# SeanNaren/deepspeech.pytorch

Measured on AMD Instinct MI355X. Metric: audio-seconds/sec (train step), higher is better.
Workload: dtype bf16

## Files before the change

deepspeech/pytorch_amd/csrc/ds2_gemm8.hip:

```cpp
#include "ds2_common.h"

namespace {

typedef __attribute__((address_space(3))) void* lds_ptr_t;
typedef const __attribute__((address_space(1))) void* glb_ptr_t;

constexpr int G8_MAX_GROUPS = 6;

struct G8Problem {
  const bf16_t* A;
  const bf16_t* A2;
  const bf16_t* B;
  void* C;
  const float* bias;
  int M, N, m_split;
  long lda, lda2, ldb, ldc;
  int tiles_n, tile_end;
  int out_is_f32;
  int K, tn;
  const int* rows;
};
struct G8Args {
  G8Problem p[G8_MAX_GROUPS];
  int n_problems;
};

#define G8_WAIT_VM(n) asm volatile("s_waitcnt vmcnt(" #n ")" ::: "memory")
#define G8_WAIT_LGKM0() asm volatile("s_waitcnt lgkmcnt(0)" ::: "memory")
#define G8_BARRIER()                        \
  do {                                      \
    __builtin_amdgcn_sched_barrier(0);      \
    __builtin_amdgcn_s_barrier();           \
    __builtin_amdgcn_sched_barrier(0);      \
  } while (0)

template <bool TN, bool SPREAD>
__device__ __forceinline__ void g8_tile(const G8Problem& P, int t_id, unsigned char* lds) {
  const int tid = threadIdx.x, lane = tid & 63;
  const int wave = __builtin_amdgcn_readfirstlane(tid >> 6);
  const int wm = wave >> 2, wn = wave & 3;
#ifndef DS2_G8_SWZ
#define DS2_G8_SWZ 1
#endif
  int tm_ = t_id / P.tiles_n, tn_ = t_id % P.tiles_n;
  if (DS2_G8_SWZ > 1 && P.tiles_n > 32 / DS2_G8_SWZ) {
    const int tiles_m = ((TN ? P.M : P.M) + 255) / 256;
    const int per = DS2_G8_SWZ * P.tiles_n, st = t_id / per, wi = t_id - st * per;
    const int rows = min(DS2_G8_SWZ, tiles_m - st * DS2_G8_SWZ);
    tm_ = st * DS2_G8_SWZ + wi % rows;
    tn_ = wi / rows;
  }
  const int m0 = tm_ * 256, n0 = tn_ * 256;
  const int K_ = P.K;
  const int nkt = (K_ + 63) / 64;
  const int krem = K_ - (nkt - 1) * 64;
  const bool tail = TN && krem < 64;

  ds2_f32x16 acc[4][2];
#pragma unroll
  for (int i = 0; i < 4; ++i)
#pragma unroll
    for (int j = 0; j < 2; ++j)
#pragma unroll
      for (int r = 0; r < 16; ++r) acc[i][j][r] = 0.f;

  uint32_t a_off[4], b_off[4];
  const bf16_t* a_base = P.A;
  const bf16_t* b_base = P.B;
  if constexpr (!TN) {
    const int rloc = wave * 8 + (lane >> 3);
    const int chunk = (lane & 7) ^ ((rloc >> 1) & 7);
#pragma unroll
    for (int rb = 0; rb < 4; ++rb) {
      int ar = min(m0 + rb * 64 + rloc, P.M - 1);
      if (P.rows) ar = P.rows[ar];
      a_off[rb] = (uint32_t)(((long)ar * P.lda + chunk * 8) * 2);
      b_off[rb] = (uint32_t)(((long)min(n0 + rb * 64 + rloc, P.N - 1) * P.ldb + chunk * 8) * 2);
    }
  } else {
#pragma unroll
    for (int rb = 0; rb < 4; ++rb) {
      const int kr = rb * 16 + wave * 2 + (lane >> 5);
      const int chunk = (lane & 31) ^ ((kr & 3) << 2);
      int mcol = m0 + chunk * 8, ncol = min(n0 + chunk * 8, P.N - 8);
      const int mlim = (P.A2 && m0 >= P.m_split) ? P.M - P.m_split : (P.A2 ? P.m_split : P.M);
      if (P.A2 && m0 >= P.m_split) mcol -= P.m_split;
      mcol = min(mcol, mlim - 8);
      a_off[rb] = (uint32_t)(((long)kr * ((P.A2 && m0 >= P.m_split) ? P.lda2 : P.lda) + mcol) * 2);
      b_off[rb] = (uint32_t)(((long)kr * P.ldb + ncol) * 2);
    }
    if (P.A2 && m0 >= P.m_split) a_base = P.A2;
  }
  const long lda_eff = (TN && P.A2 && m0 >= P.m_split) ? P.lda2 : P.lda;
  const int t_kr0 = wave * 2 + (lane >> 5);
  const uint32_t t_acol = TN ? a_off[0] - (uint32_t)((long)t_kr0 * ((P.A2 && m0 >= P.m_split) ? P.lda2 : P.lda) * 2) : 0;
  const uint32_t t_bcol = TN ? b_off[0] - (uint32_t)((long)t_kr0 * P.ldb * 2) : 0;
  const long a_kstep = TN ? 128 * lda_eff : 128, b_kstep = TN ? 128 * P.ldb : 128;
  const bool listed = TN && P.rows != nullptr;
  typedef const __attribute__((address_space(4))) int* const_int_ptr_t;
  const const_int_ptr_t crows = (const_int_ptr_t)(uintptr_t)P.rows;
  uint32_t rk[4] = {0, 0, 0, 0};
  int sr0[4] = {0, 0, 0, 0}, sr1[4] = {0, 0, 0, 0};
  auto fetch_rows = [&](int kt) {
    if (listed && kt < nkt) {
#pragma unroll
      for (int rb = 0; rb < 4; ++rb) {
        const int k = kt * 64 + rb * 16 + wave * 2;
        sr0[rb] = crows[min(k, K_ - 1)];
        sr1[rb] = crows[min(k + 1, K_ - 1)];
      }
    }
  };
  auto select_rows = [&]() {
    if (listed) {
#pragma unroll
      for (int rb = 0; rb < 4; ++rb) rk[rb] = (uint32_t)((lane >> 5) ? sr1[rb] : sr0[rb]);
    }
  };
  const uint32_t lda2b = (uint32_t)(lda_eff * 2), ldb2b = (uint32_t)(P.ldb * 2);
  auto stage_a = [&](int b, int kt, int r0 = 0, int r1 = 4) {
    const unsigned char* src = (const unsigned char*)a_base + (long)kt * a_kstep;
    unsigned char* d = lds + b * 32768 + wave * 1024;
    if (listed) {
#pragma unroll
      for (int rb = 0; rb < 4; ++rb)
        if (rb >= r0 && rb < r1)
          __builtin_amdgcn_global_load_lds((glb_ptr_t)((const unsigned char*)a_base + (size_t)(rk[rb] * lda2b + t_acol)), (lds_ptr_t)(d + rb * 8192), 16, 0, 0);
    } else if (tail && kt == nkt - 1) {
#pragma unroll
      for (int rb = 0; rb < 4; ++rb)
        if (rb >= r0 && rb < r1) {
          const uint32_t off = (uint32_t)((long)min(t_kr0 + rb * 16, krem - 1) * lda_eff * 2) + t_acol;
          __builtin_amdgcn_global_load_lds((glb_ptr_t)(src + (size_t)off), (lds_ptr_t)(d + rb * 8192), 16, 0, 0);
        }
    } else {
#pragma unroll
      for (int rb = 0; rb < 4; ++rb)
        if (rb >= r0 && rb < r1) __builtin_amdgcn_global_load_lds((glb_ptr_t)(src + (size_t)a_off[rb]), (lds_ptr_t)(d + rb * 8192), 16, 0, 0);
    }
  };
  auto stage_b = [&](int b, int kt, int r0 = 0, int r1 = 4) {
    const unsigned char* src = (const unsigned char*)b_base + (long)kt * b_kstep;
    unsigned char* d = lds + 65536 + b * 32768 + wave * 1024;
    if (listed) {
#pragma unroll
      for (int rb = 0; rb < 4; ++rb)
        if (rb >= r0 && rb < r1)
          __builtin_amdgcn_global_load_lds((glb_ptr_t)((const unsigned char*)b_base + (size_t)(rk[rb] * ldb2b + t_bcol)), (lds_ptr_t)(d + rb * 8192), 16, 0, 0);
    } else if (tail && kt == nkt - 1) {
#pragma unroll
      for (int rb = 0; rb < 4; ++rb)
        if (rb >= r0 && rb < r1) {
          const uint32_t off = (uint32_t)((long)min(t_kr0 + rb * 16, krem - 1) * P.ldb * 2) + t_bcol;
          __builtin_amdgcn_global_load_lds((glb_ptr_t)(src + (size_t)off), (lds_ptr_t)(d + rb * 8192), 16, 0, 0);
        }
    } else {
#pragma unroll
      for (int rb = 0; rb < 4; ++rb)
        if (rb >= r0 && rb < r1) __builtin_amdgcn_global_load_lds((glb_ptr_t)(src + (size_t)b_off[rb]), (lds_ptr_t)(d + rb * 8192), 16, 0, 0);
    }
  };
  auto zero_tail = [&](int b) {
    if (wm == 0) {
      const int nbytes = (64 - krem) * 512;
      for (int o = tid * 16; o < nbytes; o += 256 * 16) {
        *reinterpret_cast<uint4*>(lds + b * 32768 + krem * 512 + o) = make_uint4(0, 0, 0, 0);
        *reinterpret_cast<uint4*>(lds + 65536 + b * 32768 + krem * 512 + o) = make_uint4(0, 0, 0, 0);
      }
      G8_WAIT_LGKM0();
    }
    G8_BARRIER();
  };

  const int li = lane & 31, lq = lane >> 5;
  const uint32_t lds0 = (uint32_t)(uintptr_t)(__attribute__((address_space(3))) unsigned char*)lds;
  struct Frag {
    uint4 v;
    uint2 lo, hi;
  };
  Frag fa[2][4], fbx[4], fby[4];
  uint32_t ra[4], rb_[4];
  if constexpr (!TN) {
    const int key = (li >> 1) & 7;
#pragma unroll
    for (int c = 0; c < 4; ++c) {
      ra[c] = lds0 + (wm * 128 + li) * 128 + (((2 * c + lq) ^ key) << 4);
      rb_[c] = lds0 + 65536 + (wn * 64 + li) * 128 + (((2 * c + lq) ^ key) << 4);
    }
  } else {
    const int l16 = lane & 15, gq = lane >> 4;
    const int krow = 8 * (gq >> 1) + (l16 >> 2);
    const int mloc = 16 * (gq & 1) + 4 * (l16 & 3);
#pragma unroll
    for (int j = 0; j < 4; ++j) ra[j] = lds0 + krow * 512 + mloc * 2 + ((((wm * 4 + j) ^ (l16 >> 2))) << 6);
#pragma unroll
    for (int j = 0; j < 2; ++j) rb_[j] = lds0 + 65536 + krow * 512 + mloc * 2 + ((((wn * 2 + j) ^ (l16 >> 2))) << 6);
    rb_[2] = rb_[3] = 0;
  }
#define G8_RD128(dst, addr, off) asm volatile("ds_read_b128 %0, %1 offset:%2" : "=v"(dst) : "v"(addr), "i"(off))
#define G8_RDTR(dst, addr, off) asm volatile("ds_read_b64_tr_b16 %0, %1 offset:%2" : "=v"(dst) : "v"(addr), "i"(off))
#define G8_READ_A(BUF, MH)                                                                      \
  _Pragma("unroll") for (int i = 0; i < 2; ++i) _Pragma("unroll") for (int c = 0; c < 4; ++c) { \
    if constexpr (!TN) {                                                                        \
      G8_RD128(fa[i][c].v, ra[c], (BUF) * 32768 + ((MH) * 64 + i * 32) * 128);                  \
    } else {                                                                                    \
      G8_RDTR(fa[i][c].lo, ra[(MH) * 2 + i], (BUF) * 32768 + c * 8192);                         \
      G8_RDTR(fa[i][c].hi, ra[(MH) * 2 + i], (BUF) * 32768 + c * 8192 + 2048);                  \
    }                                                                                           \
  }
#define G8_READ_B(BUF, NH, FB)                                           \
  _Pragma("unroll") for (int c = 0; c < 4; ++c) {                        \
    if constexpr (!TN) {                                                 \
      G8_RD128(FB[c].v, rb_[c], (BUF) * 32768 + (NH) * 32 * 128);        \
    } else {                                                             \
      G8_RDTR(FB[c].lo, rb_[NH], (BUF) * 32768 + c * 8192);              \
      G8_RDTR(FB[c].hi, rb_[NH], (BUF) * 32768 + c * 8192 + 2048);       \
    }                                                                    \
  }
  auto frag = [&](const Frag& f) {
    if constexpr (!TN)
      return f.v;
    else
      return make_uint4(f.lo.x, f.lo.y, f.hi.x, f.hi.y);
  };
  auto mma = [&](int mh, int nh, const Frag (&fb)[4]) {
    __builtin_amdgcn_s_setprio(1);
#pragma unroll
    for (int c = 0; c < 4; ++c)
#pragma unroll
      for (int i = 0; i < 2; ++i)
        Mma<bf16_t>::mma32(acc[mh * 2 + i][nh], frag(fb[c]), frag(fa[i][c]));
    __builtin_amdgcn_s_setprio(0);
  };

#define G8_KTILE(BUF, KT)                                      \
  {                                                            \
    const bool more = (KT) + 2 < nkt;                          \
    const bool more_a = SPREAD && (KT) >= 1 && (KT) + 1 < nkt; \
    if (tail && (KT) == nkt - 1) zero_tail(BUF);               \
                                                  \
    fetch_rows((KT) + 2);                                      \
    G8_READ_A(BUF, 0)                                          \
    G8_READ_B(BUF, 0, fbx)                                     \
    if (more_a) stage_a((BUF) ^ 1, (KT) + 1, 0, 2);            \
    G8_BARRIER();                                              \
    G8_WAIT_LGKM0();                                           \
    __builtin_amdgcn_sched_barrier(0);                         \
    mma(0, 0, fbx);                                            \
    G8_BARRIER();                                              \
                                                  \
    G8_READ_B(BUF, 1, fby)                                     \
    if (more_a) stage_a((BUF) ^ 1, (KT) + 1, 2, 4);            \
    G8_WAIT_LGKM0();                                           \
    G8_BARRIER();                                              \
    mma(0, 1, fby);                                            \
    G8_BARRIER();                                              \
                                                  \
    G8_READ_A(BUF, 1)                                          \
    select_rows();                                             \
    if (more) stage_b(BUF, (KT) + 2, 0, SPREAD ? 2 : 4);       \
    G8_WAIT_LGKM0();                                           \
    G8_BARRIER();                                              \
    mma(1, 1, fby);                                            \
    G8_BARRIER();                                              \
                                                  \
    if (SPREAD) {                                              \
      if (more) {                                              \
        stage_b(BUF, (KT) + 2, 2, 4);                          \
        G8_WAIT_VM(4);                                         \
      } else {                                                 \
        G8_WAIT_VM(0);                                         \
      }                                                        \
    } else if (more) {                                         \
      stage_a(BUF, (KT) + 2);                                  \
      G8_WAIT_VM(8);                                           \
    } else {                                                   \
      G8_WAIT_VM(0);                                           \
    }                                                          \
    G8_BARRIER();                                              \
    mma(1, 0, fbx);                                            \
    G8_BARRIER();                                              \
  }

  fetch_rows(0);
  select_rows();
  stage_a(0, 0);
  stage_b(0, 0);
  if (nkt > 1) {
    fetch_rows(1);
    select_rows();
    stage_a(1, 1);
    stage_b(1, 1);
    G8_WAIT_VM(8);
  } else {
    G8_WAIT_VM(0);
  }
  G8_BARRIER();
  if (wm == 1) G8_BARRIER();
  for (int kt = 0; kt < nkt; kt += 2) {
    G8_KTILE(0, kt)
    if (kt + 1 < nkt) G8_KTILE(1, kt + 1)
  }
  if (wm == 0) G8_BARRIER();

  int eli = li, elq = lq;
  asm volatile("" : "+v"(eli), "+v"(elq));
  const float* bias = P.bias;
  const int M_ = P.M, N_ = P.N;
  const long ldc = P.ldc;
  if (!P.out_is_f32 && (ldc % 8 == 0) && ((((uintptr_t)P.C) & 15) == 0)) {
    unsigned char* ep = lds + wave * 9216;
    bf16_t* Cb = (bf16_t*)P.C;
#pragma unroll
    for (int half = 0; half < 2; ++half) {
#pragma unroll
      for (int i2 = 0; i2 < 2; ++i2)
#pragma unroll
        for (int j = 0; j < 2; ++j)
#pragma unroll
          for (int q = 0; q < 4; ++q) {
            const int col = j * 32 + 8 * q + 4 * elq;
            const int gcol = n0 + wn * 64 + col;
            float bv[4] = {0.f, 0.f, 0.f, 0.f};
            if (bias) {
#pragma unroll
              for (int e = 0; e < 4; ++e) bv[e] = gcol + e < N_ ? bias[gcol + e] : 0.f;
            }
            uint2 pk;
            pk.x = cvt_pk_bf16(acc[half * 2 + i2][j][4 * q + 0] + bv[0], acc[half * 2 + i2][j][4 * q + 1] + bv[1]);
            pk.y = cvt_pk_bf16(acc[half * 2 + i2][j][4 * q + 2] + bv[2], acc[half * 2 + i2][j][4 * q + 3] + bv[3]);
            *reinterpret_cast<uint2*>(ep + (i2 * 32 + eli) * 144 + col * 2) = pk;
          }
#pragma unroll
      for (int r = 0; r < 8; ++r) {
        const int row_l = r * 8 + (lane >> 3), seg = lane & 7;
        const uint4 d = *reinterpret_cast<const uint4*>(ep + row_l * 144 + seg * 16);
        const int grow = m0 + wm * 128 + half * 64 + row_l, gcol = n0 + wn * 64 + seg * 8;
        if (grow < M_) {
          bf16_t* cp = Cb + (long)(P.rows ? P.rows[grow] : grow) * ldc + gcol;
          if (gcol + 7 < N_) {
            *reinterpret_cast<uint4*>(cp) = d;
          } else {
            const uint32_t w[4] = {d.x, d.y, d.z, d.w};
#pragma unroll
            for (int e = 0; e < 8; ++e)
              if (gcol + e < N_) cp[e].v = (uint16_t)(w[e >> 1] >> ((e & 1) * 16));
          }
        }
      }
    }
    return;
  }
  const bool n_vec_ok = (ldc % 4 == 0);
#pragma unroll
  for (int i = 0; i < 4; ++i) {
    const int row = m0 + wm * 128 + i * 32 + eli;
    if (row >= M_) continue;
#pragma unroll
    for (int j = 0; j < 2; ++j) {
#pragma unroll
      for (int q = 0; q < 4; ++q) {
        const int col = n0 + wn * 64 + j * 32 + 8 * q + 4 * elq;
        if (col >= N_) continue;
        float v[4];
#pragma unroll
        for (int e = 0; e < 4; ++e) v[e] = acc[i][j][4 * q + e] + ((bias && col + e < N_) ? bias[col + e] : 0.f);
        const long off = (long)((!TN && P.rows) ? P.rows[row] : row) * ldc + col;
        if (P.out_is_f32) {
          float* cp = (float*)P.C + off;
          if (col + 3 < N_ && n_vec_ok) {
            *reinterpret_cast<float4*>(cp) = make_float4(v[0], v[1], v[2], v[3]);
          } else {
#pragma unroll
            for (int e = 0; e < 4; ++e)
              if (col + e < N_) cp[e] = v[e];
          }
        } else {
          bf16_t* cp = (bf16_t*)P.C + off;
#pragma unroll
          for (int e = 0; e < 4; ++e)
            if (col + e < N_) stf(cp + e, v[e]);
        }
      }
    }
  }
}


template <int MODE, bool SPREAD>
__global__ void __launch_bounds__(512, 2) k_gemm8(G8Args g) {
  __shared__ __attribute__((aligned(1024))) unsigned char lds[131072];
  const int id = blockIdx.x;
  int pi = 0, first = 0;
#pragma unroll
  for (int i = 0; i < G8_MAX_GROUPS - 1; ++i)
    if (i + 1 < g.n_problems && id >= g.p[i].tile_end) {
      pi = i + 1;
      first = g.p[i].tile_end;
    }
  const G8Problem& P = g.p[pi];
  const int count = P.tile_end - first, local = id - first, xcd = id & 7;
  int base = 0;
#pragma unroll
  for (int y = 0; y < 8; ++y) {
    const int l0 = (y - first) & 7;
    const int n_y = l0 < count ? (count - l0 - 1) / 8 + 1 : 0;
    if (y < xcd) base += n_y;
  }
  const int t_id = base + (local - ((xcd - first) & 7)) / 8;
  if (MODE == 0)
    g8_tile<false, SPREAD>(P, t_id, lds);
  else if (MODE == 1)
    g8_tile<true, SPREAD>(P, t_id, lds);
  else if (P.tn)
    g8_tile<true, SPREAD>(P, t_id, lds);
  else
    g8_tile<false, SPREAD>(P, t_id, lds);
}

template <int MODE>
void g8_launch(int total, const G8Args& g, hipStream_t st) {
  hipLaunchKernelGGL((k_gemm8<MODE, false>), dim3(total), dim3(512), 0, st, g);
}

}


static int g8_nt(const void* A, const void* B, void* C, const float* bias, int M, int N, int K, long lda, long ldb, long ldc, int out_f32,
                 const int* rows, int n_phys, hipStream_t st) {
  DS2_REQUIRE(M > 0 && N > 0 && K > 0 && K % 64 == 0 && lda % 8 == 0 && ldb % 8 == 0 && n_phys >= M, DS2_ERR_ARG);
  DS2_REQUIRE((((uintptr_t)A) & 15) == 0 && (((uintptr_t)B) & 15) == 0, DS2_ERR_ALIGN);
  DS2_REQUIRE((long)n_phys * lda < (1L << 31) && (long)N * ldb < (1L << 31), DS2_ERR_ARG);
  G8Args g{};
  g.n_problems = 1;
  const int tm = ds2_cdiv(M, 256), tn = ds2_cdiv(N, 256);
  g.p[0] = G8Problem{(const bf16_t*)A, nullptr, (const bf16_t*)B, C, bias, M, N, 0, lda, 0, ldb, ldc, tn, tm * tn, out_f32, K, 0, rows};
  g8_launch<0>(tm * tn, g, st);
  DS2_CHECK_LAUNCH();
  return 0;
}

static int g8_tn_fill(G8Args& g, int& total, int n, const void* const* At, const void* const* At2, const int* m_split, const void* const* Bt,
                      void* const* C, const int* M, const int* N, const long* lda, const long* lda2, const long* ldb, const long* ldc, int K,
                      const int* rows, int n_phys) {
  DS2_REQUIRE(K > 0 && n_phys >= K, DS2_ERR_ARG);
  for (int i = 0; i < n; ++i) {
    DS2_REQUIRE(M[i] > 0 && N[i] > 0 && M[i] % 8 == 0 && N[i] % 8 == 0 && lda[i] % 8 == 0 && ldb[i] % 8 == 0, DS2_ERR_ARG);
    DS2_REQUIRE((((uintptr_t)At[i]) & 15) == 0 && (((uintptr_t)Bt[i]) & 15) == 0, DS2_ERR_ALIGN);
    DS2_REQUIRE((long)n_phys * lda[i] < (1L << 31) && (long)n_phys * ldb[i] < (1L << 31), DS2_ERR_ARG);
    const void* a2 = At2 ? At2[i] : nullptr;
    const int ms = a2 ? m_split[i] : 0;
    DS2_REQUIRE(a2 == nullptr || (ms > 0 && ms < M[i] && ms % 256 == 0 && (((uintptr_t)a2) & 15) == 0 && lda2 && lda2[i] % 8 == 0 &&
                                  (long)n_phys * lda2[i] < (1L << 31)), DS2_ERR_ARG);
    const int tm = ds2_cdiv(M[i], 256), tn = ds2_cdiv(N[i], 256);
    total += tm * tn;
    g.p[i] = G8Problem{(const bf16_t*)At[i], (const bf16_t*)a2, (const bf16_t*)Bt[i], C[i], nullptr, M[i], N[i], ms, lda[i], a2 ? lda2[i] : 0, ldb[i], ldc[i], tn, total, 1, K, 1, rows};
  }
  return 0;
}

extern "C" {

int ds2_gemm8_nt(const void* A, const void* B, void* C, const float* bias, int M, int N, int K, long lda, long ldb, long ldc, int out_f32,
                 ds2_stream_t st) {
  return g8_nt(A, B, C, bias, M, N, K, lda, ldb, ldc, out_f32, nullptr, M, (hipStream_t)st);
}
int ds2_gemm8_nt_rows(const void* A, const void* B, void* C, const float* bias, int n_phys, int N, int K, long lda, long ldb, long ldc,
                      int out_f32, const int* rows, int n_rows, ds2_stream_t st) {
  return g8_nt(A, B, C, bias, rows ? n_rows : n_phys, N, K, lda, ldb, ldc, out_f32, rows, n_phys, (hipStream_t)st);
}

int ds2_gemm8_tn_grouped_rows(int n_problems, const void* const* At, const void* const* At2, const int* m_split, const void* const* Bt,
                              void* const* C, const int* M, const int* N, const long* lda, const long* lda2, const long* ldb, const long* ldc,
                              int n_phys, const int* rows, int n_rows, ds2_stream_t st) {
  DS2_REQUIRE(n_problems >= 1 && n_problems <= G8_MAX_GROUPS, DS2_ERR_ARG);
  G8Args g{};
  g.n_problems = n_problems;
  int total = 0;
  const int rc = g8_tn_fill(g, total, n_problems, At, At2, m_split, Bt, C, M, N, lda, lda2, ldb, ldc, rows ? n_rows : n_phys, rows, n_phys);
  if (rc) return rc;
  g8_launch<1>(total, g, (hipStream_t)st);
  DS2_CHECK_LAUNCH();
  return 0;
}
int ds2_gemm8_tn_grouped(int n_problems, const void* const* At, const void* const* At2, const int* m_split, const void* const* Bt, void* const* C,
                         const int* M, const int* N, const long* lda, const long* lda2, const long* ldb, const long* ldc, int K, ds2_stream_t st) {
  return ds2_gemm8_tn_grouped_rows(n_problems, At, At2, m_split, Bt, C, M, N, lda, lda2, ldb, ldc, K, nullptr, K, st);
}

int ds2_gemm8_wgrad_dx_rows(int n_tn, const void* const* At, const void* const* At2, const int* m_split, const void* const* Bt, void* const* C,
                            const int* M, const int* N, const long* lda, const long* lda2, const long* ldb, const long* ldc, int K_tn,
                            const void* A_nt, const void* B_nt, void* C_nt, int M_nt, int N_nt, int K_nt, long lda_nt, long ldb_nt, long ldc_nt,
                            const int* rows, int n_rows, ds2_stream_t st) {
  DS2_REQUIRE(n_tn >= 1 && n_tn < G8_MAX_GROUPS && K_tn > 0, DS2_ERR_ARG);
  DS2_REQUIRE(rows == nullptr || (K_tn == M_nt && n_rows > 0 && n_rows <= K_tn), DS2_ERR_ARG);
  DS2_REQUIRE(M_nt > 0 && N_nt > 0 && K_nt > 0 && K_nt % 64 == 0 && lda_nt % 8 == 0 && ldb_nt % 8 == 0, DS2_ERR_ARG);
  DS2_REQUIRE((((uintptr_t)A_nt) & 15) == 0 && (((uintptr_t)B_nt) & 15) == 0, DS2_ERR_ALIGN);
  DS2_REQUIRE((long)M_nt * lda_nt < (1L << 31) && (long)N_nt * ldb_nt < (1L << 31), DS2_ERR_ARG);
  G8Args g{};
  g.n_problems = n_tn + 1;
  int total = 0;
  const int rc = g8_tn_fill(g, total, n_tn, At, At2, m_split, Bt, C, M, N, lda, lda2, ldb, ldc, rows ? n_rows : K_tn, rows, K_tn);
  if (rc) return rc;
  const int m_eff = rows ? n_rows : M_nt;
  const int tm = ds2_cdiv(m_eff, 256), tn = ds2_cdiv(N_nt, 256);
  total += tm * tn;
  g.p[n_tn] = G8Problem{(const bf16_t*)A_nt, nullptr, (const bf16_t*)B_nt, C_nt, nullptr, m_eff, N_nt, 0, lda_nt, 0, ldb_nt, ldc_nt, tn, total, 0, K_nt, 0, rows};
  g8_launch<2>(total, g, (hipStream_t)st);
  DS2_CHECK_LAUNCH();
  return 0;
}
int ds2_gemm8_wgrad_dx(int n_tn, const void* const* At, const void* const* At2, const int* m_split, const void* const* Bt, void* const* C,
                       const int* M, const int* N, const long* lda, const long* lda2, const long* ldb, const long* ldc, int K_tn,
                       const void* A_nt, const void* B_nt, void* C_nt, int M_nt, int N_nt, int K_nt, long lda_nt, long ldb_nt, long ldc_nt,
                       ds2_stream_t st) {
  return ds2_gemm8_wgrad_dx_rows(n_tn, At, At2, m_split, Bt, C, M, N, lda, lda2, ldb, ldc, K_tn, A_nt, B_nt, C_nt, M_nt, N_nt, K_nt, lda_nt,
                                 ldb_nt, ldc_nt, nullptr, 0, st);
}

}
```

Measured before the change: 21390.

## Load B fragments directly from global into registers for NT GEMM path

For the non-transposed path, B operand tiles are no longer staged through LDS. Each wave loads its B fragments straight from global memory into double-buffered registers, one k-tile ahead, while A still goes through LDS. The aim is to remove LDS write/read traffic and the barriers tied to B staging. In exchange it raises VGPR pressure, drops the tail zeroing and row-gather handling on this path, and relies on hand-tuned vmcnt waits.

```diff
diff --git a/deepspeech/pytorch_amd/csrc/ds2_gemm8.hip b/deepspeech/pytorch_amd/csrc/ds2_gemm8.hip
--- a/deepspeech/pytorch_amd/csrc/ds2_gemm8.hip
+++ b/deepspeech/pytorch_amd/csrc/ds2_gemm8.hip
@@ -4,6 +4,7 @@
 
 typedef __attribute__((address_space(3))) void* lds_ptr_t;
 typedef const __attribute__((address_space(1))) void* glb_ptr_t;
+typedef uint32_t g8_u32x4 __attribute__((ext_vector_type(4)));
 
 constexpr int G8_MAX_GROUPS = 6;
 
@@ -75,7 +76,7 @@
       int ar = min(m0 + rb * 64 + rloc, P.M - 1);
       if (P.rows) ar = P.rows[ar];
       a_off[rb] = (uint32_t)(((long)ar * P.lda + chunk * 8) * 2);
-      b_off[rb] = (uint32_t)(((long)min(n0 + rb * 64 + rloc, P.N - 1) * P.ldb + chunk * 8) * 2);
+      b_off[rb] = 0;
     }
   } else {
 #pragma unroll
@@ -179,6 +180,12 @@
     uint2 lo, hi;
   };
   Frag fa[2][4], fbx[4], fby[4];
+  Frag fbg[2][2][4];
+  uint32_t bg_off[2] = {0, 0};
+  if constexpr (!TN) {
+#pragma unroll
+    for (int j = 0; j < 2; ++j) bg_off[j] = (uint32_t)(((long)min(n0 + wn * 64 + j * 32 + li, P.N - 1) * P.ldb + lq * 8) * 2);
+  }
   uint32_t ra[4], rb_[4];
   if constexpr (!TN) {
     const int key = (li >> 1) & 7;
@@ -232,6 +239,54 @@
         Mma<bf16_t>::mma32(acc[mh * 2 + i][nh], frag(fb[c]), frag(fa[i][c]));
     __builtin_amdgcn_s_setprio(0);
   };
+
+#define G8_GLD128(dst, voff, sbase, off) asm volatile("global_load_dwordx4 %0, %1, %2 offset:%3" : "=v"(dst) : "v"(voff), "s"(sbase), "i"(off))
+#define G8_LOAD_B(SET, KT, J)                                                                  \
+  {                                                                                            \
+    const unsigned char* sb_ = (const unsigned char*)b_base + (long)min((KT), nkt - 1) * 128;  \
+    _Pragma("unroll") for (int c = 0; c < 4; ++c) G8_GLD128(fbg[SET][J][c].v, bg_off[J], sb_, c * 32); \
+  }
+#define G8_PIN_B(F) asm volatile("" : "+v"(*(g8_u32x4*)&F[0].v), "+v"(*(g8_u32x4*)&F[1].v), "+v"(*(g8_u32x4*)&F[2].v), "+v"(*(g8_u32x4*)&F[3].v))
+#define G8_KTILE_NT(BUF, KT)                                                   \
+  {                                                                            \
+    const bool next = (KT) + 1 < nkt, more = (KT) + 2 < nkt;                   \
+                     \
+    G8_READ_A(BUF, 0)                                                          \
+    G8_LOAD_B((BUF) ^ 1, (KT) + 1, 0)                                          \
+    G8_BARRIER();                                                              \
+    G8_WAIT_LGKM0();                                                           \
+    if (next) G8_WAIT_VM(12); else G8_WAIT_VM(8);                              \
+    G8_PIN_B(fbg[BUF][0]);                                                     \
+    __builtin_amdgcn_sched_barrier(0);                                         \
+    mma(0, 0, fbg[BUF][0]);                                                    \
+    G8_BARRIER();                                                              \
+                   \
+    G8_LOAD_B((BUF) ^ 1, (KT) + 1, 1)                                          \
+    G8_BARRIER();                                                              \
+    if (next) G8_WAIT_VM(12); else G8_WAIT_VM(8);                              \
+    G8_PIN_B(fbg[BUF][1]);                                                     \
+    __builtin_amdgcn_sched_barrier(0);                                         \
+    mma(0, 1, fbg[BUF][1]);                                                    \
+    G8_BARRIER();                                                              \
+                                                                  \
+    G8_READ_A(BUF, 1)                                                          \
+    G8_WAIT_LGKM0();                                                           \
+    G8_BARRIER();                                                              \
+    mma(1, 1, fbg[BUF][1]);                                                    \
+    G8_BARRIER();                                                              \
+     \
+    if (more) {                                                                \
+      stage_a(BUF, (KT) + 2);                                                  \
+      G8_WAIT_VM(12);                                                          \
+    } else if (next) {                                                         \
+      G8_WAIT_VM(8);                                                           \
+    } else {                                                                   \
+      G8_WAIT_VM(0);                                                           \
+    }                                                                          \
+    G8_BARRIER();                                                              \
+    mma(1, 0, fbg[BUF][0]);                                                    \
+    G8_BARRIER();                                                              \
+  }
 
 #define G8_KTILE(BUF, KT)                                      \
   {                                                            \
@@ -282,6 +337,24 @@
     G8_BARRIER();                                              \
   }
 
+  if constexpr (!TN) {
+    stage_a(0, 0);
+    G8_LOAD_B(0, 0, 0)
+    G8_LOAD_B(0, 0, 1)
+    if (nkt > 1) {
+      stage_a(1, 1);
+      G8_WAIT_VM(12);
+    } else {
+      G8_WAIT_VM(8);
+    }
+    G8_BARRIER();
+    if (wm == 1) G8_BARRIER();
+    for (int kt = 0; kt < nkt; kt += 2) {
+      G8_KTILE_NT(0, kt)
+      if (kt + 1 < nkt) G8_KTILE_NT(1, kt + 1)
+    }
+    if (wm == 0) G8_BARRIER();
+  } else {
   fetch_rows(0);
   select_rows();
   stage_a(0, 0);
@@ -302,6 +375,7 @@
     if (kt + 1 < nkt) G8_KTILE(1, kt + 1)
   }
   if (wm == 0) G8_BARRIER();
+  }
 
   int eli = li, elq = lq;
   asm volatile("" : "+v"(eli), "+v"(elq));
```

Measured after the change: 20490. 0.958x the previous value.
